# JonathonLuiten/PReMVOS

Measured on AMD Instinct MI355X. Metric: frames/sec (proposal+refine+flow) on 480p DAVIS frames, higher is better.
Workload: dtype f32

## Files before the change

include/premvos_hip.h:

```cpp
#ifndef PREMVOS_HIP_H
#define PREMVOS_HIP_H

#include <stdint.h>

#ifdef __cplusplus
extern "C" {
#endif

#define PREMVOS_OK 0
#define PREMVOS_EINVAL (-1)
#define PREMVOS_ELAUNCH (-2)
#define PREMVOS_EUNSUPPORTED (-3)
#define PREMVOS_ENOSPACE (-4)

#define PREMVOS_ACT_NONE 0
#define PREMVOS_ACT_RELU 1
#define PREMVOS_ACT_LEAKY 2
#define PREMVOS_ACT_SIGMOID 3
#define PREMVOS_ACT_SPLIT8_BF16 0x200

#define PREMVOS_PREC_F32 0
#define PREMVOS_PREC_BF16 1
#define PREMVOS_PREC_BF16X3 3

// ... 37 lines not shown
} premvos_conv_desc;

int premvos_conv2d_f32(const premvos_conv_desc* d, void* stream);
int64_t premvos_conv2d_workspace_bytes(const premvos_conv_desc* d);

int premvos_conv_wino4_slab_f32(const premvos_conv_desc* d, float* vslab, int64_t vslab_bytes, int32_t v_pitch, int32_t v_c0, int32_t t_cn,
                                void* stream);

int premvos_corr_fwd_f32(const float* f1, int32_t f1_ps, const float* f2, int32_t f2_ps, float* out,
                         int32_t out_ps, int32_t n, int32_t h, int32_t w, int32_t c, int32_t md,
                         float slope, int32_t copy_f1, void* stream);

int premvos_corr_nchw_fwd_f32(const float* in1, const float* in2, float* out, int32_t n, int32_t c,
                              int32_t h, int32_t w, int32_t pad_size, int32_t kernel_size,
                              int32_t max_displacement, int32_t stride1, int32_t stride2,
                              int32_t corr_type_multiply, void* stream);

int premvos_warp_fwd_f32(const float* x, int32_t x_ps, const float* flow, int32_t flow_ps, float flow_scale,
                         float* out, int32_t out_ps, int32_t n, int32_t h, int32_t w, int32_t c,
                         void* stream);

int premvos_warp_corr_fwd_f32(const float* f1, int32_t f1_ps, const float* x2, int32_t x2_ps, const float* flow,
                              int32_t flow_ps, float flow_scale, float* out, int32_t out_ps, int32_t n, int32_t h,
                              int32_t w, int32_t c, int32_t md, float slope, int32_t copy_f1, void* stream);

int premvos_nchw_to_nhwc_f32(const float* in, float* out, int32_t out_ps, int32_t n, int32_t c, int32_t h,
                             int32_t w, void* stream);
int premvos_nhwc_to_nchw_f32(const float* in, int32_t in_ps, float* out, int32_t n, int32_t c, int32_t h,
                             int32_t w, void* stream);

int premvos_flow_preprocess_u8(const uint8_t* im1, const uint8_t* im2, int32_t batch, int32_t h, int32_t w,
                               float* out, int32_t h_, int32_t w_, void* stream);
int premvos_flow_postprocess_f32(const float* flow2, int32_t flow_ps, int32_t batch, int32_t h4, int32_t w4,
                                 float* out, int32_t h, int32_t w, int32_t h_, int32_t w_, void* stream);


int premvos_proposal_preprocess_u8(const uint8_t* img_bgr, int32_t batch, int32_t h, int32_t w, float* out,
                                   int32_t nh, int32_t nw, int32_t src_is_rgb, void* stream);

int premvos_maxpool_f32(const float* in, int32_t in_ps, int32_t n, int32_t h, int32_t w, int32_t c, float* out,
                        int32_t out_ps, int32_t ho, int32_t wo, int32_t k, int32_t stride, int32_t pt, int32_t pl,
                        float pad_value, void* stream);

int premvos_rpn_proposals_f32(const float* rpn, int32_t ps, int32_t n, int32_t fh, int32_t fw, int32_t na,
                              int32_t logit_off, int32_t box_off, const float* cell_anchors, float stride,
                              float img_h, float img_w, int32_t pre_nms_topk, int32_t post_nms_topk,
                              float nms_thresh, float min_size, float decode_clip, float* out_boxes,
                              float* out_scores, int32_t* out_idx, int32_t* out_count, void* stream);

int premvos_roi_align_f32(const float* fmap, int32_t fmap_ps, int32_t n_img, int32_t h, int32_t w, int32_t c,
                          const float* rois, const int32_t* count, int32_t rois_per_img, float spatial_scale,
                          int32_t out_size, float* out, int32_t out_ps, void* stream);

int premvos_global_avgpool_f32(const float* in, int32_t in_ps, int32_t n, int32_t hw, int32_t c, float* out,
                               int32_t out_ps, void* stream);

int premvos_frcnn_tail_f32(const float* head, int32_t head_ps, const float* rois, const int32_t* count, int32_t n_img,
                           int32_t rois_per_img, float img_h, float img_w, float score_thresh, float nms_thresh,
                           int32_t max_out, float decode_clip, float rw_x, float rw_y, float rw_w, float rw_h,
                           float* out_boxes, float* out_probs, int32_t* out_idx, int32_t* out_count, void* stream);


int premvos_refine_input_u8(const uint8_t* frame_rgb, int32_t h, int32_t w, const float* boxes_y0x0y1x1,
                            const int32_t* count, int32_t max_boxes, int32_t size, float* out, int32_t* crop_boxes,
                            void* stream);

int premvos_dwconv3x3_f32(const float* in, int32_t in_ps, int32_t n, int32_t h, int32_t w, int32_t c,
                          const float* wgt, const float* bias, int32_t c_pad, float* out, int32_t out_ps, int32_t ho,
                          int32_t wo, int32_t stride, int32_t dilation, int32_t pt, int32_t pl, int32_t pre_relu,
                          int32_t act, void* stream);

#define PREMVOS_DW_TILE 1
#define PREMVOS_DW_ROW 2
#define PREMVOS_DW_PIXEL 3
#define PREMVOS_DW_STORE_F32 0
#define PREMVOS_DW_STORE_S8 1
#define PREMVOS_DW_STORE_S8_PAIRED 2
int premvos_dwconv3x3_variant(int32_t n, int32_t h, int32_t w, int32_t c_pad, int32_t ho, int32_t wo, int32_t stride,
                              int32_t dilation, int32_t pre_relu, int32_t act);

int premvos_conv_bf16x3_s8_f32(const premvos_conv_desc* d, const void* in_s8, const void* wgt_s8, void* out_s8,
                               int32_t out_s8_ps, const void* res_s8, int32_t res_s8_ps, int32_t tile, void* stream);

int premvos_split8_f32(const float* in, int32_t in_ps, void* out_s8, int32_t out_ps, int64_t pixels, int32_t c, void* stream);

int premvos_resize_bilinear_f32(const float* in, int32_t in_ps, int32_t n, int32_t h, int32_t w, int32_t c, float* out,
                                int32_t out_ps, int32_t ho, int32_t wo, int32_t align_corners, void* stream);

int premvos_broadcast_pixel_f32(const float* in, int32_t in_ps, int32_t n, int32_t c, float* out, int32_t out_ps,
                                int32_t h, int32_t w, void* stream);

int64_t premvos_refine_output_workspace_bytes(int32_t max_boxes, int32_t size, int32_t h, int32_t w);
int premvos_refine_output_f32(const float* logits, int32_t logits_ps, int32_t lh, int32_t lw, const int32_t* crop_boxes,
                              const int32_t* count, int32_t max_boxes, int32_t size, int32_t h, int32_t w,
                              uint8_t* mask, float* posterior, float* conf_score, void* workspace, void* stream);

int premvos_mfma_f32_calibrate(int64_t iters, int32_t blocks, float* sink, void* stream);

int premvos_mfma_f32_calibrate_random(int64_t iters, int32_t blocks, float* sink, void* stream);

int premvos_hbm_copy_calibrate(const void* src, void* dst, int64_t n_float4, void* stream);

int premvos_digest_u64(const void* buf, int64_t pixels, int32_t c, int32_t ps, void* out_u64, void* stream);

uint32_t premvos_crc32c_host(const void* data, int64_t n);

// ... 165 lines not shown
```

premvos_amd/_lib.py:

```python
from __future__ import annotations

import ctypes as C
import os

import torch

from . import build as _build

_LIB = None
ABI_VERSION = 21

ACT_NONE, ACT_RELU, ACT_LEAKY, ACT_SIGMOID = 0, 1, 2, 3
MASK_BBOX_SLABS = 16
ACT_SPLIT8_BF16 = 0x200
OUT_NHWC, OUT_PIXSHUF2 = 0, 1
PREC_F32, PREC_BF16, PREC_BF16X3 = 0, 1, 3
PRECISIONS = {"fp32": PREC_F32, "bf16": PREC_BF16, "bf16x3": PREC_BF16X3}


class ConvDesc(C.Structure):
    _fields_ = [
        ("inp", C.c_void_p), ("wgt", C.c_void_p), ("bias", C.c_void_p), ("res", C.c_void_p),
        ("out", C.c_void_p),
        ("n", C.c_int32), ("h", C.c_int32), ("w", C.c_int32), ("cin", C.c_int32),
        ("in_ps", C.c_int32),
        ("ho", C.c_int32), ("wo", C.c_int32), ("cout", C.c_int32),
        ("out_ps", C.c_int32), ("res_ps", C.c_int32),
        ("kh", C.c_int32), ("kw", C.c_int32), ("sh", C.c_int32), ("sw", C.c_int32),
        ("dh", C.c_int32), ("dw", C.c_int32), ("pt", C.c_int32), ("pl", C.c_int32),
        ("cin_pad", C.c_int32), ("k_pad", C.c_int32), ("cout_pad", C.c_int32),
        ("act", C.c_int32), ("slope", C.c_float), ("out_mode", C.c_int32), ("cout_ps", C.c_int32),
        ("tile_hint", C.c_int32), ("split_k", C.c_int32), ("workspace", C.c_void_p), ("workspace_bytes", C.c_int64),
        ("precision", C.c_int32), ("stage_k", C.c_int32), ("wgt_lo", C.c_void_p),
        ("tail_m_tiles", C.c_int32), ("tail_split_k", C.c_int32), ("wgt_wino", C.c_void_p),
        ("wgt_wino4", C.c_void_p),
    ]


_i32, _f32, _vp = C.c_int32, C.c_float, C.c_void_p

SIGNATURES = {
    "premvos_conv2d_f32": [C.POINTER(ConvDesc), _vp],
    "premvos_corr_fwd_f32": [_vp, _i32, _vp, _i32, _vp, _i32, _i32, _i32, _i32, _i32, _i32, _f32, _i32, _vp],
    "premvos_corr_nchw_fwd_f32": [_vp, _vp, _vp, _i32, _i32, _i32, _i32, _i32, _i32, _i32, _i32, _i32, _i32, _vp],
    "premvos_warp_corr_fwd_f32": [_vp, _i32, _vp, _i32, _vp, _i32, _f32, _vp, _i32, _i32, _i32, _i32, _i32, _i32, _f32,
                                  _i32, _vp],
    "premvos_warp_fwd_f32": [_vp, _i32, _vp, _i32, _f32, _vp, _i32, _i32, _i32, _i32, _i32, _vp],
    "premvos_nchw_to_nhwc_f32": [_vp, _vp, _i32, _i32, _i32, _i32, _i32, _vp],
    "premvos_nhwc_to_nchw_f32": [_vp, _i32, _vp, _i32, _i32, _i32, _i32, _vp],
    "premvos_flow_preprocess_u8": [_vp, _vp, _i32, _i32, _i32, _vp, _i32, _i32, _vp],
    "premvos_flow_postprocess_f32": [_vp, _i32, _i32, _i32, _i32, _vp, _i32, _i32, _i32, _i32, _vp],
    "premvos_proposal_preprocess_u8": [_vp, _i32, _i32, _i32, _vp, _i32, _i32, _i32, _vp],
    "premvos_maxpool_f32": [_vp, _i32, _i32, _i32, _i32, _i32, _vp, _i32, _i32, _i32, _i32, _i32, _i32, _i32, _f32, _vp],
    "premvos_rpn_proposals_f32": [_vp, _i32, _i32, _i32, _i32, _i32, _i32, _i32, _vp, _f32, _f32, _f32, _i32, _i32,
                                  _f32, _f32, _f32, _vp, _vp, _vp, _vp, _vp],
    "premvos_roi_align_f32": [_vp, _i32, _i32, _i32, _i32, _i32, _vp, _vp, _i32, _f32, _i32, _vp, _i32, _vp],
    "premvos_global_avgpool_f32": [_vp, _i32, _i32, _i32, _i32, _vp, _i32, _vp],
    "premvos_refine_input_u8": [_vp, _i32, _i32, _vp, _vp, _i32, _i32, _vp, _vp, _vp],
    "premvos_dwconv3x3_f32": [_vp, _i32, _i32, _i32, _i32, _i32, _vp, _vp, _i32, _vp, _i32, _i32, _i32, _i32, _i32,
                              _i32, _i32, _i32, _i32, _vp],
    "premvos_conv_bf16x3_s8_f32": [C.POINTER(ConvDesc), _vp, _vp, _vp, _i32, _vp, _i32, _i32, _vp],
    "premvos_split8_f32": [_vp, _i32, _vp, _i32, C.c_int64, _i32, _vp],
    "premvos_resize_bilinear_f32": [_vp, _i32, _i32, _i32, _i32, _i32, _vp, _i32, _i32, _i32, _i32, _vp],
    "premvos_broadcast_pixel_f32": [_vp, _i32, _i32, _i32, _vp, _i32, _i32, _i32, _vp],
    "premvos_refine_output_f32": [_vp, _i32, _i32, _i32, _vp, _vp, _i32, _i32, _i32, _i32, _vp, _vp, _vp, _vp, _vp],
    "premvos_mfma_f32_calibrate": [C.c_int64, _i32, _vp, _vp],
    "premvos_mfma_f32_calibrate_random": [C.c_int64, _i32, _vp, _vp],
    "premvos_hbm_copy_calibrate": [_vp, _vp, C.c_int64, _vp],
    "premvos_digest_u64": [_vp, C.c_int64, _i32, _i32, _vp, _vp],
    "premvos_conv_wino4_slab_f32": [C.POINTER(ConvDesc), _vp, C.c_int64, _i32, _i32, _i32, _vp],
    "premvos_jpeg_entropy_decode_host": [_vp, C.c_int64, _vp, _vp, C.c_int64],
    "premvos_jpeg_reconstruct_u8": [_vp, _vp, _vp, _vp, _i32, _vp],
    "premvos_overlay_blend_u8": [_vp, _vp, _vp, _i32, _i32, _vp, _vp],
    "premvos_jpeg_forward_u8": [_vp, _vp, _vp, _i32, _i32, _vp, _vp, _i32, _i32, _vp, _vp, C.c_int64, _vp],
    "premvos_jpeg_entropy_encode_host": [_vp, _vp, _vp, C.c_int64, _vp],
    "premvos_reid_input_u8": [_vp, _i32, _i32, _vp, _i32, _i32, _i32, _vp, _vp],
    "premvos_reid_input_frames_u8": [_vp, _i32, _i32, _i32, _vp, _vp, _i32, _i32, _i32, _vp, _vp],
    "premvos_reid_context_boxes_i32": [_vp, _i32, _i32, _i32, _i32, _vp, _vp],
    "premvos_mask_bbox_u8": [_vp, _i32, _i32, _i32, C.c_int64, _i32, _i32, _vp, _vp, _vp, _vp],
    "premvos_scale_shift_relu_f32": [_vp, _i32, C.c_int64, _i32, _vp, _vp, _vp, _i32, _i32, _vp],
    "premvos_mask_warp_u8": [_vp, _i32, _i32, _i32, _vp, _vp, _i32, _vp],
    "premvos_mask_overlap_u8": [_vp, _i32, _vp, _i32, C.c_int64, _vp, _vp, _vp, _vp],
    "premvos_mask_warp_seats_u8": [_vp, _i32, _i32, _i32, _vp, _vp, _i32, _vp, _i32, _vp],
    "premvos_mask_pack_bits_u8": [_vp, C.c_int64, _vp, _vp],
    "premvos_mask_unpack_bits_u8": [_vp, C.c_int64, _vp, _vp],
    "premvos_rle_boundaries_u8": [_vp, _i32, _i32, _i32, _vp, _i32, _vp, _vp, _vp],
    "premvos_rle_boundaries_pooled_u8": [_vp, _i32, _i32, _i32, C.c_int64, _i32, _vp, _i32, _vp, _vp, _vp],
    "premvos_frcnn_tail_f32": [_vp, _i32, _vp, _vp, _i32, _i32, _f32, _f32, _f32, _f32, _i32, _f32, _f32, _f32, _f32,
                               _f32, _vp, _vp, _vp, _vp, _vp],
    "premvos_rle_decode_u8": [_vp, _i32, _vp, _i32, _i32, _i32, _vp, _vp],
    "premvos_track_scores_f64": [_vp, _vp, _vp, _vp, _vp, _vp, _vp, _i32, _i32, _vp, C.c_double, _vp, _vp, _vp, _vp, _vp, _vp],
    "premvos_track_paint_u8": [_vp, _i32, _i32, _i32, _vp, _vp, _vp, _i32, _vp, _vp, _vp, _vp],
    "premvos_track_inputs_f64": [_vp, _vp, _vp, _vp, _i32, _i32, _vp, _vp, _vp],
    "premvos_track_next_f32": [_vp, _vp, _i32, _vp, _vp, _vp],
    "premvos_mask_overlap_seats_u8": [_vp, _i32, C.c_int64, _vp, _i32, _vp, _vp, _vp, _vp],
    "premvos_track_scores_seats_f64": [_vp, _vp, _vp, _vp, _vp, _vp, _vp, _vp, _vp, _i32, _vp, C.c_double, _vp, _vp, _vp, _vp, _vp, _vp],
    "premvos_track_paint_seats_u8": [_vp, _i32, _i32, _i32, _vp, _i32, _vp, _vp, _vp, _vp, _vp, _vp, _i32, _vp, _vp],
    "premvos_track_scores_sets_f64": [_vp, _vp, _vp, _vp, _vp, _vp, _vp, _vp, _vp, _i32, _vp, C.c_double, _vp, _vp, _vp, _vp, _vp, _vp],
    "premvos_track_eval_seats_i64": [_vp, _i32, _i32, _i32, _vp, _i32, _i32, _vp, _vp, C.c_int64, _vp],
    "premvos_mask_label_overlap_u8": [_vp, _i32, _vp, _i32, C.c_int64, _vp, _vp, _vp, _vp],
    "premvos_track_gt_scores_f64": [_vp, _vp, _vp, _i32, _i32, _vp, C.c_double, _vp, _vp, _vp, _vp, _vp, _vp],
    "premvos_track_combine_f64": [_vp, _i32, _i32, _i32, _vp, C.c_int64, _vp, _i32, _vp, _vp, _vp, _vp, _vp, _vp, _vp],
    "premvos_viz_scores_u8": [_vp, _i32, _i32, _vp, _vp, _i32, _vp, _vp, C.c_int64, _vp, _i32, _vp, _vp, C.c_int64, _vp, _vp],
    "premvos_reid_max_distance_f64": [_vp, _i32, _vp, C.c_int64, _vp, _vp, _vp],
    "premvos_davis_counts_u8":[_vp, _vp, _i32, _i32, _i32, _vp, _i32, _i32, _vp, _vp, _vp],
    "premvos_bits_overlap_i32": [_vp, _i32, C.c_int64, C.c_int64, _vp, _vp, _i32, _vp, C.c_int64, _vp, C.c_int64, _vp],
    "premvos_prewarp_reid_f64": [_vp, _vp, _i32, _i32, _vp, _vp, _i32, _vp, _vp, _vp, _vp, _vp],
    "premvos_prewarp_chain_f64": [_vp, C.c_int64, _vp, C.c_int64, _vp, _vp, _vp, _vp, _vp, _vp, _i32, _i32, _vp, _vp, _vp, _vp, _i32, _vp, _vp,
                                  _vp, _vp],
# ... 100 lines not shown
```

premvos_amd/csrc/proposal_ops.hip:

```cpp
#include "common.h"
#include "resize_cv.h"

#pragma clang fp contract(off)

namespace {

__global__ __launch_bounds__(256) void proposal_preprocess_kernel(const uint8_t* __restrict__ img, int batch, int h,
                                                                  int w, float* __restrict__ out, int nh, int nw,
                                                                  int src_is_rgb) {
  const long total = (long)batch * nh * nw;
  const double sx = 1.0 / ((double)nw / (double)w), sy = 1.0 / ((double)nh / (double)h);
  const float mean[3] = {0.406f, 0.456f, 0.485f};
  const float stdv[3] = {0.225f, 0.224f, 0.229f};
  const float inv255 = (float)(1.0 / 255);
  for (long idx = (long)blockIdx.x * 256 + threadIdx.x; idx < total; idx += (long)gridDim.x * 256) {
    const int x = idx % nw, y = (idx / nw) % nh;
    const uint8_t* im = img + (idx / ((long)nw * nh)) * h * w * 3;
    int x0, x1, y0, y1;
    short a0, a1, b0, b1;
    premvos::cv_lin_coef(x, sx, w, &x0, &x1, &a0, &a1);
    premvos::cv_lin_coef(y, sy, h, &y0, &y1, &b0, &b1);
    float px[4];
    for (int ch = 0; ch < 3; ++ch) {
      const int sc = src_is_rgb ? 2 - ch : ch;
// ... 265 lines not shown
    if (rl < count[img]) {
      const float* rb = rois + r * 4;
      const float x0 = rb[0] * scale, y0 = rb[1] * scale, x1 = rb[2] * scale, y1 = rb[3] * scale;
      const float sw = (x1 - x0) / (float)crop, sh = (y1 - y0) / (float)crop;
      const float nx0 = (x0 + sw / 2.f - 0.5f) / (float)(W - 1), ny0 = (y0 + sh / 2.f - 0.5f) / (float)(H - 1);
      const float nw = sw * (float)(crop - 1) / (float)(W - 1), nh = sh * (float)(crop - 1) / (float)(H - 1);
      const float by1 = ny0, bx1 = nx0, by2 = ny0 + nh, bx2 = nx0 + nw;
      const float hs = (by2 - by1) * (float)(H - 1) / (float)(crop - 1);
      const float ws = (bx2 - bx1) * (float)(W - 1) / (float)(crop - 1);
      const float* fb = fm + (long)img * H * W * ps + cg * 4;
      bool oky[2], okx[2];
      int yt[2], yb[2], xl[2], xr[2];
      float yl[2], xlp[2];
#pragma unroll
      for (int j = 0; j < 2; ++j) {
        const float in_y = by1 * (float)(H - 1) + (float)(2 * by_ + j) * hs;
        oky[j] = !(in_y < 0.f || in_y > (float)(H - 1));
        yt[j] = (int)floorf(in_y), yb[j] = (int)ceilf(in_y);
        yl[j] = in_y - floorf(in_y);
        const float in_x = bx1 * (float)(W - 1) + (float)(2 * bx_ + j) * ws;
        okx[j] = !(in_x < 0.f || in_x > (float)(W - 1));
        xl[j] = (int)floorf(in_x), xr[j] = (int)ceilf(in_x);
        xlp[j] = in_x - floorf(in_x);
      }
      float4 tl[2][2], tr[2][2], bl[2][2], br[2][2];
#pragma unroll
      for (int j = 0; j < 2; ++j)
#pragma unroll
        for (int i = 0; i < 2; ++i)
          if (oky[j] && okx[i]) {
            tl[j][i] = *reinterpret_cast<const float4*>(fb + ((long)yt[j] * W + xl[i]) * ps);
            tr[j][i] = *reinterpret_cast<const float4*>(fb + ((long)yt[j] * W + xr[i]) * ps);
            bl[j][i] = *reinterpret_cast<const float4*>(fb + ((long)yb[j] * W + xl[i]) * ps);
            br[j][i] = *reinterpret_cast<const float4*>(fb + ((long)yb[j] * W + xr[i]) * ps);
          }
#pragma unroll
      for (int j = 0; j < 2; ++j)
#pragma unroll
        for (int i = 0; i < 2; ++i)
          if (oky[j] && okx[i]) {
            const float4 a = tl[j][i], b = tr[j][i], c = bl[j][i], d = br[j][i];
            float top, bot;
            top = a.x + (b.x - a.x) * xlp[i]; bot = c.x + (d.x - c.x) * xlp[i]; acc.x += top + (bot - top) * yl[j];
            top = a.y + (b.y - a.y) * xlp[i]; bot = c.y + (d.y - c.y) * xlp[i]; acc.y += top + (bot - top) * yl[j];
            top = a.z + (b.z - a.z) * xlp[i]; bot = c.z + (d.z - c.z) * xlp[i]; acc.z += top + (bot - top) * yl[j];
            top = a.w + (b.w - a.w) * xlp[i]; bot = c.w + (d.w - c.w) * xlp[i]; acc.w += top + (bot - top) * yl[j];
          }
      acc.x *= 0.25f; acc.y *= 0.25f; acc.z *= 0.25f; acc.w *= 0.25f;
    }
    *reinterpret_cast<float4*>(out + ((r * outsz + by_) * outsz + bx_) * out_ps + cg * 4) = acc;
  }
}

__global__ __launch_bounds__(256) void roi_align_row_kernel(const float* __restrict__ fm, int ps, int H, int W, int c4,
                                                            const float* __restrict__ rois, const int* __restrict__ count,
                                                            int rois_per_img, int n_img, float scale, int outsz,
                                                            float* __restrict__ out, int out_ps) {
  const long total = (long)n_img * rois_per_img * outsz * c4;
  const int crop = 2 * outsz;
  for (long idx = (long)blockIdx.x * 256 + threadIdx.x; idx < total; idx += (long)gridDim.x * 256) {
    const int cg = idx % c4;
    long t = idx / c4;
    const int by_ = t % outsz;
    const long r = t / outsz;
    const int img = r / rois_per_img, rl = r % rois_per_img;
    float* orow = out + ((r * outsz + by_) * outsz) * out_ps + cg * 4;
    if (rl >= count[img]) {
      for (int bx_ = 0; bx_ < outsz; ++bx_) *reinterpret_cast<float4*>(orow + (long)bx_ * out_ps) = make_float4(0.f, 0.f, 0.f, 0.f);
      continue;
    }
    const float* rb = rois + r * 4;
    const float x0 = rb[0] * scale, y0 = rb[1] * scale, x1 = rb[2] * scale, y1 = rb[3] * scale;
    const float sw = (x1 - x0) / (float)crop, sh = (y1 - y0) / (float)crop;
    const float nx0 = (x0 + sw / 2.f - 0.5f) / (float)(W - 1), ny0 = (y0 + sh / 2.f - 0.5f) / (float)(H - 1);
    const float nw = sw * (float)(crop - 1) / (float)(W - 1), nh = sh * (float)(crop - 1) / (float)(H - 1);
    const float by1 = ny0, bx1 = nx0, by2 = ny0 + nh, bx2 = nx0 + nw;
    const float hs = (by2 - by1) * (float)(H - 1) / (float)(crop - 1);
    const float ws = (bx2 - bx1) * (float)(W - 1) / (float)(crop - 1);
    const float* fb = fm + (long)img * H * W * ps + cg * 4;
    bool oky[2];
    float yl[2];
    const float* rt[2];
    const float* rbt[2];
#pragma unroll
    for (int j = 0; j < 2; ++j) {
      const float in_y = by1 * (float)(H - 1) + (float)(2 * by_ + j) * hs;
      oky[j] = !(in_y < 0.f || in_y > (float)(H - 1));
      const int yt = oky[j] ? (int)floorf(in_y) : 0, yb = oky[j] ? (int)ceilf(in_y) : 0;
      yl[j] = in_y - floorf(in_y);
      rt[j] = fb + (long)yt * W * ps;
      rbt[j] = fb + (long)yb * W * ps;
    }
    float4 L[2][2], R[2][2];
    int cxl = -2, cxr = -2;
    float4 sv[2][2];
    bool sok[2];
    for (int bx_ = 0; bx_ < outsz; ++bx_) {
#pragma unroll
      for (int i = 0; i < 2; ++i) {
        const int sx = 2 * bx_ + i;
        const float in_x = bx1 * (float)(W - 1) + (float)sx * ws;
        const bool okx = !(in_x < 0.f || in_x > (float)(W - 1));
        sok[i] = okx;
        if (okx) {
          const int xl = (int)floorf(in_x), xr = (int)ceilf(in_x);
          const float xlp = in_x - floorf(in_x);
          if (xl != cxl || xr != cxr) {
            const bool shift = xl == cxr;
#pragma unroll
            for (int j = 0; j < 2; ++j)
              if (oky[j]) {
                if (shift) { L[j][0] = R[j][0]; L[j][1] = R[j][1]; }
                else {
                  L[j][0] = *reinterpret_cast<const float4*>(rt[j] + (long)xl * ps);
                  L[j][1] = *reinterpret_cast<const float4*>(rbt[j] + (long)xl * ps);
                }
                if (xr == xl) { R[j][0] = L[j][0]; R[j][1] = L[j][1]; }
                else {
                  R[j][0] = *reinterpret_cast<const float4*>(rt[j] + (long)xr * ps);
                  R[j][1] = *reinterpret_cast<const float4*>(rbt[j] + (long)xr * ps);
                }
              }
            cxl = xl; cxr = xr;
          }
#pragma unroll
          for (int j = 0; j < 2; ++j)
            if (oky[j]) {
              const float4 a = L[j][0], b = R[j][0], c = L[j][1], d = R[j][1];
              float top, bot;
              top = a.x + (b.x - a.x) * xlp; bot = c.x + (d.x - c.x) * xlp; sv[j][i].x = top + (bot - top) * yl[j];
              top = a.y + (b.y - a.y) * xlp; bot = c.y + (d.y - c.y) * xlp; sv[j][i].y = top + (bot - top) * yl[j];
              top = a.z + (b.z - a.z) * xlp; bot = c.z + (d.z - c.z) * xlp; sv[j][i].z = top + (bot - top) * yl[j];
              top = a.w + (b.w - a.w) * xlp; bot = c.w + (d.w - c.w) * xlp; sv[j][i].w = top + (bot - top) * yl[j];
            }
        }
      }
      float4 acc = make_float4(0.f, 0.f, 0.f, 0.f);
#pragma unroll
      for (int j = 0; j < 2; ++j)
#pragma unroll
        for (int ii = 0; ii < 2; ++ii)
          if (oky[j] && sok[ii]) { acc.x += sv[j][ii].x; acc.y += sv[j][ii].y; acc.z += sv[j][ii].z; acc.w += sv[j][ii].w; }
      acc.x *= 0.25f; acc.y *= 0.25f; acc.z *= 0.25f; acc.w *= 0.25f;
      *reinterpret_cast<float4*>(orow + (long)bx_ * out_ps) = acc;
    }
  }
}

__global__ __launch_bounds__(256) void gap_kernel(const float* __restrict__ in, int in_ps, int n, int hw, int c4,
                                                  float* __restrict__ out, int out_ps) {
  const long total = (long)n * c4;
  for (long idx = (long)blockIdx.x * 256 + threadIdx.x; idx < total; idx += (long)gridDim.x * 256) {
    const int cg = idx % c4;
    const long b = idx / c4;
    float4 s = make_float4(0.f, 0.f, 0.f, 0.f);
    for (int i = 0; i < hw; ++i) {
      const float4 v = *reinterpret_cast<const float4*>(in + (b * hw + i) * in_ps + cg * 4);
      s.x += v.x; s.y += v.y; s.z += v.z; s.w += v.w;
    }
    const float inv = (float)hw;
    *reinterpret_cast<float4*>(out + b * out_ps + cg * 4) = make_float4(s.x / inv, s.y / inv, s.z / inv, s.w / inv);
  }
}

__global__ __launch_bounds__(256) void gap_sliced_kernel(const float* __restrict__ in, int in_ps, int hw, int c4,
                                                         float* __restrict__ out, int out_ps) {
  __shared__ float4 part[8][32];
  const int lane = threadIdx.x & 31, slice = threadIdx.x >> 5;
  const int cg = blockIdx.x * 32 + lane;
  const long b = blockIdx.y;
  float4 s = make_float4(0.f, 0.f, 0.f, 0.f);
  if (cg < c4) {
    const float* base = in + b * hw * (long)in_ps + cg * 4;
    for (int i = slice; i < hw; i += 8) {
      const float4 v = *reinterpret_cast<const float4*>(base + (long)i * in_ps);
      s.x += v.x; s.y += v.y; s.z += v.z; s.w += v.w;
    }
  }
  part[slice][lane] = s;
  __syncthreads();
  if (slice == 0 && cg < c4) {
#pragma unroll
    for (int k = 1; k < 8; ++k) {
      const float4 v = part[k][lane];
      s.x += v.x; s.y += v.y; s.z += v.z; s.w += v.w;
    }
    const float inv = (float)hw;
    *reinterpret_cast<float4*>(out + b * out_ps + cg * 4) = make_float4(s.x / inv, s.y / inv, s.z / inv, s.w / inv);
  }
}

constexpr int TAIL_NT = 128;

struct TailArgs {
  const float* head;
  int ps, rois_per_img;
  const float* rois;
// ... 85 lines not shown
}

extern "C" int premvos_maxpool_f32(const float* in, int32_t in_ps, int32_t n, int32_t h, int32_t w, int32_t c,
                                   float* out, int32_t out_ps, int32_t ho, int32_t wo, int32_t k, int32_t stride,
                                   int32_t pt, int32_t pl, float pad_value, void* stream) {
  PV_REQUIRE(in && out, "maxpool: null pointer");
  PV_REQUIRE(n > 0 && h > 0 && w > 0 && c > 0 && ho > 0 && wo > 0 && k > 0 && stride > 0, "maxpool: bad dims");
  PV_REQUIRE(c % 4 == 0 && in_ps % 4 == 0 && out_ps % 4 == 0 && in_ps >= c && out_ps >= c,
             "maxpool: C and pixel strides must be multiples of 4");
  PV_REQUIRE(premvos::aligned16(in) && premvos::aligned16(out), "maxpool: in/out must be 16-byte aligned");
  hipLaunchKernelGGL(maxpool_kernel, dim3(grid_for((long)n * ho * wo * (c / 4))), dim3(256), 0,
                     static_cast<hipStream_t>(stream), in, in_ps, n, h, w, c / 4, out, out_ps, ho, wo, k, stride, pt,
                     pl, pad_value);
  return premvos::check_launch("maxpool");
}

extern "C" int premvos_rpn_proposals_f32(const float* rpn, int32_t ps, int32_t n, int32_t fh, int32_t fw, int32_t na,
                                         int32_t logit_off, int32_t box_off, const float* cell_anchors, float stride,
                                         float img_h, float img_w, int32_t pre_nms_topk, int32_t post_nms_topk,
                                         float nms_thresh, float min_size, float decode_clip, float* out_boxes,
                                         float* out_scores, int32_t* out_idx, int32_t* out_count, void* stream) {
  PV_REQUIRE(rpn && cell_anchors && out_boxes && out_scores && out_idx && out_count, "rpn_proposals: null pointer");
  PV_REQUIRE(n > 0 && fh > 0 && fw > 0 && na > 0, "rpn_proposals: bad dims");
  PV_REQUIRE(ps >= logit_off + na && ps >= box_off + 4 * na && logit_off >= 0 && box_off >= 0,
             "rpn_proposals: channel window exceeds pixel stride");
  PV_REQUIRE(pre_nms_topk > 0 && pre_nms_topk <= RPN_NT, "rpn_proposals: pre_nms_topk must be in [1,%d]", RPN_NT);
  PV_REQUIRE(post_nms_topk > 0 && post_nms_topk <= 128, "rpn_proposals: post_nms_topk must be in [1,128]");
  PV_REQUIRE((long)fh * fw * na < (1L << 31), "rpn_proposals: too many anchors");
  RpnArgs a;
  a.rpn = rpn; a.ps = ps; a.fh = fh; a.fw = fw; a.na = na; a.logit_off = logit_off; a.box_off = box_off;
  a.cell_anchors = cell_anchors; a.stride = stride; a.img_h = img_h; a.img_w = img_w; a.nms_thresh = nms_thresh;
  a.min_size = min_size; a.decode_clip = decode_clip; a.pre_k = pre_nms_topk; a.post_k = post_nms_topk;
  a.out_boxes = out_boxes; a.out_scores = out_scores; a.out_idx = out_idx; a.out_count = out_count;
  hipLaunchKernelGGL(rpn_proposals_kernel, dim3(n), dim3(RPN_NT), 0, static_cast<hipStream_t>(stream), a);
  return premvos::check_launch("rpn_proposals");
}

extern "C" int premvos_roi_align_f32(const float* fmap, int32_t fmap_ps, int32_t n_img, int32_t h, int32_t w,
                                     int32_t c, const float* rois, const int32_t* count, int32_t rois_per_img,
                                     float spatial_scale, int32_t out_size, float* out, int32_t out_ps, void* stream) {
  PV_REQUIRE(fmap && rois && count && out, "roi_align: null pointer");
  PV_REQUIRE(n_img > 0 && h > 1 && w > 1 && c > 0 && rois_per_img > 0 && out_size > 0, "roi_align: bad dims");
  PV_REQUIRE(c % 4 == 0 && fmap_ps % 4 == 0 && out_ps % 4 == 0 && fmap_ps >= c && out_ps >= c,
             "roi_align: C and pixel strides must be multiples of 4");
  PV_REQUIRE(premvos::aligned16(fmap) && premvos::aligned16(out), "roi_align: fmap/out must be 16-byte aligned");
  static const bool per_bin = [] { const char* e = getenv("PREMVOS_ROI_ALIGN"); return e != nullptr && e[0] == 'b'; }();
  if (per_bin) {
    const long total = (long)n_img * rois_per_img * out_size * out_size * (c / 4);
    hipLaunchKernelGGL(roi_align_kernel, dim3(grid_for(total)), dim3(256), 0,
                       static_cast<hipStream_t>(stream), fmap, fmap_ps, h, w, c / 4, rois, count, rois_per_img, n_img,
                       spatial_scale, out_size, out, out_ps);
  } else {
    const long total = (long)n_img * rois_per_img * out_size * (c / 4);
    hipLaunchKernelGGL(roi_align_row_kernel, dim3(grid_for(total)), dim3(256), 0,
                       static_cast<hipStream_t>(stream), fmap, fmap_ps, h, w, c / 4, rois, count, rois_per_img, n_img,
                       spatial_scale, out_size, out, out_ps);
  }
  return premvos::check_launch("roi_align");
}

extern "C" int premvos_global_avgpool_f32(const float* in, int32_t in_ps, int32_t n, int32_t hw, int32_t c, float* out,
                                          int32_t out_ps, void* stream) {
  PV_REQUIRE(in && out, "global_avgpool: null pointer");
  PV_REQUIRE(n > 0 && hw > 0 && c > 0, "global_avgpool: bad dims");
  PV_REQUIRE(c % 4 == 0 && in_ps % 4 == 0 && out_ps % 4 == 0 && in_ps >= c && out_ps >= c,
             "global_avgpool: C and strides must be multiples of 4");
  PV_REQUIRE(premvos::aligned16(in) && premvos::aligned16(out), "global_avgpool: in/out must be 16-byte aligned");
  if (hw >= 128) {
    hipLaunchKernelGGL(gap_sliced_kernel, dim3((c / 4 + 31) / 32, n), dim3(256), 0, static_cast<hipStream_t>(stream), in,
                       in_ps, hw, c / 4, out, out_ps);
  } else {
    hipLaunchKernelGGL(gap_kernel, dim3(grid_for((long)n * (c / 4))), dim3(256), 0, static_cast<hipStream_t>(stream),
                       in, in_ps, n, hw, c / 4, out, out_ps);
  }
  return premvos::check_launch("global_avgpool");
}

extern "C" int premvos_frcnn_tail_f32(const float* head, int32_t head_ps, const float* rois, const int32_t* count,
                                      int32_t n_img, int32_t rois_per_img, float img_h, float img_w,
                                      float score_thresh, float nms_thresh, int32_t max_out, float decode_clip,
                                      float rw_x, float rw_y, float rw_w, float rw_h, float* out_boxes,
                                      float* out_probs, int32_t* out_idx, int32_t* out_count, void* stream) {
  PV_REQUIRE(head && rois && count && out_boxes && out_probs && out_idx && out_count, "frcnn_tail: null pointer");
  PV_REQUIRE(rw_x > 0.f && rw_y > 0.f && rw_w > 0.f && rw_h > 0.f, "frcnn_tail: bad regression weights");
  PV_REQUIRE(n_img > 0 && rois_per_img > 0 && rois_per_img <= TAIL_NT, "frcnn_tail: rois_per_img must be in [1,%d]",
             TAIL_NT);
  PV_REQUIRE(head_ps >= 6 && max_out > 0 && max_out <= 64, "frcnn_tail: bad head_ps/max_out");
  TailArgs a;
  a.head = head; a.ps = head_ps; a.rois_per_img = rois_per_img; a.rois = rois; a.count = count;
  a.img_h = img_h; a.img_w = img_w; a.score_thresh = score_thresh; a.nms_thresh = nms_thresh;
  a.decode_clip = decode_clip;
  a.rw0 = rw_x; a.rw1 = rw_y; a.rw2 = rw_w; a.rw3 = rw_h;
  a.max_out = max_out; a.out_boxes = out_boxes; a.out_probs = out_probs; a.out_idx = out_idx; a.out_count = out_count;
  hipLaunchKernelGGL(frcnn_tail_kernel, dim3(n_img), dim3(TAIL_NT), 0, static_cast<hipStream_t>(stream), a);
  return premvos::check_launch("frcnn_tail");
}
```

premvos_amd/proposal/model.py:

```python
from __future__ import annotations

import math
from typing import Dict, Optional, Sequence, Tuple

import numpy as np
import torch

from .. import _lib, arena, ops
from ..ops import ACT_NONE, ACT_RELU, ACT_SIGMOID, NHWC
from ..plan import LaunchPlan

RESNET_NUM_BLOCK = (3, 4, 23, 3)
ANCHOR_STRIDE = 16
ANCHOR_SIZES = (32, 64, 128, 256, 512)
ANCHOR_RATIOS = (0.5, 1.0, 2.0)
NUM_ANCHOR = 15
MAX_SIZE = 1333
BBOX_DECODE_CLIP = float(np.float32(np.log(MAX_SIZE / 16.0)))
TEST_PRE_NMS_TOPK, TEST_POST_NMS_TOPK = 1000, 100
RPN_PROPOSAL_NMS_THRESH, RPN_MIN_SIZE = 0.7, 0.0
FASTRCNN_BBOX_REG_WEIGHTS = (10.0, 10.0, 5.0, 5.0)
FASTRCNN_NMS_THRESH, RESULT_SCORE_THRESH, RESULTS_PER_IM = 0.5, 0.5, 20
NUM_CLASS, SECOND_NUM_CLASS = 2, 81
BN_EPS = 1e-5


def cell_anchors() -> np.ndarray:
    base = ANCHOR_STRIDE
    scales = np.array(ANCHOR_SIZES, np.float64) / base
    out = []
    w = h = float(base)
    xc = yc = 0.5 * (base - 1)
    for r in ANCHOR_RATIOS:
        ws = np.round(np.sqrt(w * h / r))
        hs = np.round(ws * r)
        for s in scales:
            sw, sh = ws * s, hs * s
            out.append([xc - 0.5 * (sw - 1), yc - 0.5 * (sh - 1), xc + 0.5 * (sw - 1), yc + 0.5 * (sh - 1)])
    a = np.array(out, np.float32)
    a[:, 2:] += 1
    return a


def _fold_bn(bn: Dict[str, torch.Tensor]) -> Tuple[torch.Tensor, torch.Tensor]:
    scale = bn["gamma"].double() / torch.sqrt(bn["var"].double() + BN_EPS)
    bias = bn["beta"].double() - bn["mean"].double() * scale
    return scale.float(), bias.float()


class _Plan(LaunchPlan):
    def __init__(self, net: "ProposalNet", b: int, h: int, w: int):
        dev = net.device
        self.b, self.h, self.w = b, h, w
        self.arena = arena.two_pass(dev, lambda A: self._build(net, b, h, w, A))
        self.tune(dev)

    def _build(self, net: "ProposalNet", b: int, h: int, w: int, A: "arena.Arena"):
        self.reset()
        P, lib = net.packed, _lib.load()

        def alloc(n, hh, ww, c):
            ps = (c + 3) // 4 * 4
            return NHWC(A.alloc(n, hh, ww, ps, "f32", pooled=ps == c), c=c)

        S8 = net.packed_s8

        def alloc_s8(n, hh, ww, c):
            assert c % 8 == 0
            return NHWC(A.alloc(n, hh, ww, c, "s8"), c=c, layout="s8")

        def release(*vs):
            for v in vs:
                if v is not None:
                    A.release(v)

        def conv(x, name, out, uid=None, **kw):
            self.conv(uid or name, x, (S8 if x.layout == "s8" else P)[name], out, **kw)

        self.img = alloc(b, h, w, 3)
        h0, w0 = ops.out_size(h, 7, 2, 2, 3), ops.out_size(w, 7, 2, 2, 3)
        c0 = alloc(b, h0, w0, 64)
        conv(self.img, "conv0", c0, stride=(2, 2), pad=(2, 2), act=ACT_RELU)
        hp, wp = ops.out_size(h0, 3, 2, 0, 1), ops.out_size(w0, 3, 2, 0, 1)
        x = alloc(b, hp, wp, 64)

        def pool(i=c0, o=x):
            _lib.check(lib.premvos_maxpool_f32(i.ptr, i.ps, i.n, i.h, i.w, i.c, o.ptr, o.ps, o.h, o.w, 3, 2, 0, 0,
                                               0.0, _lib.current_stream()), "maxpool")
        self.add("maxpool", pool)
        release(c0)

        def group(x: Optional[NHWC], g: int, feat: int, count: int, stride: int, tag: str = "", x8: Optional[NHWC] = None,
                  last_s8: bool = False, last_f32: bool = True):
            s8 = net.s8 and g >= net.s8_from
            shape = (x if x is not None else x8)
            n_, h_, w_, c_ = shape.n, shape.h, shape.w, shape.c
            own_x = own_x8 = False
            for i in range(count):
                p = f"group{g}/block{i}"
                s = stride if i == 0 else 1
                last = i + 1 == count
                if s8 and x8 is None:
                    x8 = alloc_s8(n_, h_, w_, c_)
                    own_x8 = True
                    self.add(f"split8:{tag}{p}", lambda i_=x, o_=x8: ops.split8(i_, o_))
                xin = x8 if s8 else x
                mk = alloc_s8 if s8 else alloc
                t1 = mk(n_, h_, w_, feat)
                o1 = dict(out=None, out_s8=t1) if s8 else dict(out=t1)
                conv(xin, p + "/conv1", uid=tag + p + "/conv1", act=ACT_RELU, **o1)
                if s == 2:
                    ho, wo = ops.out_size(h_, 3, 2, 0, 1), ops.out_size(w_, 3, 2, 0, 1)
                    t2 = mk(n_, ho, wo, feat)
                    o2 = dict(out=None, out_s8=t2) if s8 else dict(out=t2)
                    conv(t1, p + "/conv2", uid=tag + p + "/conv2", stride=(2, 2), pad=(0, 0), act=ACT_RELU, **o2)
                else:
                    ho, wo = h_, w_
                    t2 = mk(n_, h_, w_, feat)
                    o2 = dict(out=None, out_s8=t2) if s8 else dict(out=t2)
                    conv(t1, p + "/conv2", uid=tag + p + "/conv2", pad=(1, 1), act=ACT_RELU, **o2)
                res, res8 = x, None
                if p + "/convshortcut" in P or p + "/convshortcut" in S8:
                    res = alloc(n_, ho, wo, feat * 4)
                    conv(xin, p + "/convshortcut", res, uid=tag + p + "/convshortcut", stride=(s, s))
                elif s8:
                    res, res8 = None, x8
                want_f32 = not s8 or (last and last_f32)
                y = alloc(n_, ho, wo, feat * 4) if want_f32 else None
                y8 = alloc_s8(n_, ho, wo, feat * 4) if s8 and (not last or last_s8) else None
                conv(t2, p + "/conv3", y, uid=tag + p + "/conv3", out_s8=y8, res=res, res_s8=res8, act=ACT_RELU)
                release(t1, t2, res if res is not x else None, x if own_x else None, x8 if own_x8 else None)
                x, x8, h_, w_, c_, own_x, own_x8 = y, y8, ho, wo, feat * 4, True, True
            return x, x8

        nb = net.num_blocks
        s8g = [net.s8 and g >= net.s8_from for g in range(4)]
        x1, x18 = group(x, 0, 64, nb[0], 1, last_s8=s8g[1], last_f32=not s8g[1])
        release(x)
        x2, x28 = group(x1, 1, 128, nb[1], 2, x8=x18, last_s8=s8g[2], last_f32=not s8g[2])
        release(x1, x18)
        fm, fm8 = group(x2, 2, 256, nb[2], 2, x8=x28, last_s8=net.s8 and net.s8_rpn)
        release(x2, x28)
        self.featuremap = fm
        fh, fw = fm.h, fm.w
        hid = alloc(b, fh, fw, 1024)
        conv(fm8 if fm8 is not None else fm, "rpn/conv0", hid, pad=(1, 1), act=ACT_RELU)
        release(fm8)
        self.rpn_out = alloc(b, fh, fw, 5 * NUM_ANCHOR)
        conv(hid, "rpn/heads", self.rpn_out)
        release(hid)
        R = TEST_POST_NMS_TOPK
        self.rois = A.side((b, R, 4), torch.float32)
        self.roi_scores = A.side((b, R), torch.float32)
        self.roi_idx = A.side((b, R), torch.int32)
        self.roi_count = A.side((b,), torch.int32)
        ca = net.cell_anchors_dev

        def rpn(o=self.rpn_out):
            _lib.check(lib.premvos_rpn_proposals_f32(
                o.ptr, o.ps, b, fh, fw, NUM_ANCHOR, 0, NUM_ANCHOR, ca.data_ptr(), float(ANCHOR_STRIDE), float(h),
                float(w), TEST_PRE_NMS_TOPK, R, RPN_PROPOSAL_NMS_THRESH, RPN_MIN_SIZE, BBOX_DECODE_CLIP,
                self.rois.data_ptr(), self.roi_scores.data_ptr(), self.roi_idx.data_ptr(), self.roi_count.data_ptr(),
                _lib.current_stream()), "rpn_proposals")
        self.add("rpn_proposals", rpn)
        roi = alloc(b * R, 14, 14, 1024)

        def ralign(o=roi):
            _lib.check(lib.premvos_roi_align_f32(fm.ptr, fm.ps, b, fh, fw, 1024, self.rois.data_ptr(),
                                                 self.roi_count.data_ptr(), R, 1.0 / ANCHOR_STRIDE, 14, o.ptr, o.ps,
                                                 _lib.current_stream()), "roi_align")
        self.add("roi_align", ralign)
        f5, _ = group(roi, 3, 512, nb[3], 2)
        release(roi)
        self.feat5 = f5
        gp = alloc(b * R, 1, 1, 2048)

        def gap(i=f5, o=gp):
            _lib.check(lib.premvos_global_avgpool_f32(i.ptr, i.ps, i.n, i.h * i.w, i.c, o.ptr, o.ps,
                                                      _lib.current_stream()), "gap")
        self.add("global_avgpool", gap)
        nh = NUM_CLASS + 4 * (NUM_CLASS - 1) + SECOND_NUM_CLASS
        self.head = alloc(b * R, 1, 1, nh)
        conv(gp, "heads", self.head)
        M = RESULTS_PER_IM
        self.final_boxes = A.side((b, M, 4), torch.float32)
        self.final_probs = A.side((b, M), torch.float32)
        self.final_idx = A.side((b, M), torch.int32)
        self.final_count = A.side((b,), torch.int32)

        def tail(hd=self.head):
            _lib.check(lib.premvos_frcnn_tail_f32(
                hd.ptr, hd.ps, self.rois.data_ptr(), self.roi_count.data_ptr(), b, R, float(h), float(w),
                RESULT_SCORE_THRESH, FASTRCNN_NMS_THRESH, M, BBOX_DECODE_CLIP, *FASTRCNN_BBOX_REG_WEIGHTS,
                self.final_boxes.data_ptr(), self.final_probs.data_ptr(), self.final_idx.data_ptr(),
                self.final_count.data_ptr(), _lib.current_stream()), "frcnn_tail")
        self.add("frcnn_tail", tail)

        self.final_masks: Optional[NHWC] = None
        if net.mode_mask:
            mroi = alloc(b * M, 14, 14, 1024)

            def malign(o=mroi):
                _lib.check(lib.premvos_roi_align_f32(fm.ptr, fm.ps, b, fh, fw, 1024, self.final_boxes.data_ptr(),
                                                     self.final_count.data_ptr(), M, 1.0 / ANCHOR_STRIDE, 14, o.ptr,
                                                     o.ps, _lib.current_stream()), "roi_align(mask)")
            self.add("roi_align_mask", malign)
            mf5, _ = group(mroi, 3, 512, nb[3], 2, tag="mask:")
            release(mroi)
            up = alloc(b * M, 14, 14, 256)
            conv(mf5, "maskrcnn/deconv", up, act=ACT_RELU)
            release(mf5)
            self.final_masks = alloc(b * M, 14, 14, NUM_CLASS - 1)
            conv(up, "maskrcnn/conv", self.final_masks, act=ACT_SIGMOID)
            release(up)


class ProposalNet:

    def __init__(self, weights: Dict[str, object], num_blocks: Sequence[int] = RESNET_NUM_BLOCK,
                 device=None, use_graph: bool = True, precision: Optional[str] = None,
                 mode_mask: bool = False):
        _lib.require_gpu()
        self.mode_mask = mode_mask
        self.precision = prec = precision or ops.default_precision()
        self.device, self.use_graph, self.num_blocks = _lib.resolve_device(device), use_graph, tuple(num_blocks)
        device = self.device
        self.packed: Dict[str, ops.PackedConv] = {}
        self._plans: Dict[tuple, _Plan] = {}
        self.cell_anchors_dev = torch.from_numpy(cell_anchors()).to(device)
        w = weights
        import os
        self.s8 = prec == "bf16x3" and os.environ.get("PREMVOS_BF16X3_SPLIT", "1") != "0"
        self.s8_from = int(os.environ.get("PREMVOS_BF16X3_S8_FROM", "1"))
        self.packed_s8: Dict[str, ops.PackedConvS8] = {}
        for name in [k[:-2] for k in w if k.endswith("/W") and (k[:-2] + "/bn") in w]:
            scale, bias = _fold_bn(w[name + "/bn"])
            if self.s8 and name.startswith("group") and int(name[5]) >= self.s8_from:
                self.packed_s8[name] = ops.pack_conv_s8(w[name + "/W"], bias, device, scale=scale)
            else:
                self.packed[name] = ops.pack_conv(w[name + "/W"], bias, device, scale=scale, precision="fp32" if self.s8 else prec)
        self.s8_rpn = os.environ.get("PREMVOS_S8_RPN", "0") == "1"
        if self.s8 and self.s8_rpn:
            self.packed_s8["rpn/conv0"] = ops.pack_conv_s8(w["rpn/conv0/W"], w["rpn/conv0/b"], device)
        else:
            self.packed["rpn/conv0"] = ops.pack_conv(w["rpn/conv0/W"], w["rpn/conv0/b"], device, precision="fp32" if self.s8 else prec)
        self.packed["rpn/heads"] = ops.pack_conv(torch.cat([w["rpn/class/W"], w["rpn/box/W"]], 0),
                                                 torch.cat([w["rpn/class/b"], w["rpn/box/b"]], 0), device, precision=prec)
        hw = torch.cat([w["fastrcnn/class/W"], w["fastrcnn/box/W"], w["secondclassification/class/W"]], 0)
        hb = torch.cat([w["fastrcnn/class/b"], w["fastrcnn/box/b"], w["secondclassification/class/b"]], 0)
        self.packed["heads"] = ops.pack_conv(hw.view(hw.shape[0], hw.shape[1], 1, 1), hb, device, precision=prec)
        if mode_mask:
            self.packed["maskrcnn/deconv"] = ops.pack_deconv2x2s2(w["maskrcnn/deconv/W"], w["maskrcnn/deconv/b"], device,
                                                                  precision=prec)
            self.packed["maskrcnn/conv"] = ops.pack_conv(w["maskrcnn/conv/W"], w["maskrcnn/conv/b"], device, precision=prec)

    def plan(self, b: int, h: int, w: int) -> _Plan:
        key = (b, h, w)
        if key not in self._plans:
            if h // ANCHOR_STRIDE < 2 or w // ANCHOR_STRIDE < 2:
                raise ValueError("image too small for the stride-16 feature map")
            p = _Plan(self, b, h, w)
            if self.use_graph:
                p.capture()
            self._plans[key] = p
        return self._plans[key]

    def run_resized(self, img_bgr: torch.Tensor) -> _Plan:
        b, h, w, _ = img_bgr.shape
        p = self.plan(b, h, w)
        _lib.check(_lib.load().premvos_proposal_preprocess_u8(img_bgr.contiguous().data_ptr(), b, h, w, p.img.ptr, h,
                                                              w, 0, _lib.current_stream()), "proposal_preprocess")
        p.launch()
        return p

    def outputs(self, p: _Plan, i: int = 0):
        n = int(p.final_count[i].item())
        boxes = p.final_boxes[i, :n].cpu().numpy()
        probs = p.final_probs[i, :n].cpu().numpy()
        idx = p.final_idx[i, :n].cpu().numpy().astype(np.int64)
        labels = np.ones((n,), np.int64)
        head = p.head.buf.view(p.b, TEST_POST_NMS_TOPK, -1)[i].cpu().numpy()
        cls = head[:, :2]
        e = np.exp(cls - cls.max(1, keepdims=True))
        label_probs = e / e.sum(1, keepdims=True)
        final_posterior = label_probs[np.zeros((n,), np.int64)] if n else np.zeros((0, 2), np.float32)
        sec = head[:, 6:6 + SECOND_NUM_CLASS]
        es = np.exp(sec - sec.max(1, keepdims=True))
        sec_probs = es / es.sum(1, keepdims=True)
        second_final_posterior = sec_probs[np.zeros((n,), np.int64)] if n else np.zeros((0, SECOND_NUM_CLASS), np.float32)
        second_final_labels = (final_posterior.argmax(-1) + 1) if n else np.zeros((0,), np.int64)
        return boxes, probs, labels, final_posterior, second_final_labels, second_final_posterior, idx

    def masks(self, p: _Plan, i: int = 0) -> np.ndarray:
# ... 4 lines not shown
```

Measured before the change: 54.26.

## Commute group3 block0 1x1 conv and shortcut sampling ahead of ROI align

```diff
diff --git a/include/premvos_hip.h b/include/premvos_hip.h
--- a/include/premvos_hip.h
+++ b/include/premvos_hip.h
@@ -113,6 +113,11 @@
                           const float* rois, const int32_t* count, int32_t rois_per_img, float spatial_scale,
                           int32_t out_size, float* out, int32_t out_ps, void* stream);
 
+int premvos_roi_align_epi_f32(const float* fmap, int32_t fmap_ps, int32_t n_img, int32_t h, int32_t w, int32_t c,
+                              const float* rois, const int32_t* count, int32_t rois_per_img, float spatial_scale,
+                              int32_t out_size, int32_t bin_step, const float* bias, int32_t act, float* out,
+                              int32_t out_ps, void* stream);
+
 int premvos_global_avgpool_f32(const float* in, int32_t in_ps, int32_t n, int32_t hw, int32_t c, float* out,
                                int32_t out_ps, void* stream);
 
diff --git a/premvos_amd/_lib.py b/premvos_amd/_lib.py
--- a/premvos_amd/_lib.py
+++ b/premvos_amd/_lib.py
@@ -55,6 +55,8 @@
     "premvos_rpn_proposals_f32": [_vp, _i32, _i32, _i32, _i32, _i32, _i32, _i32, _vp, _f32, _f32, _f32, _i32, _i32,
                                   _f32, _f32, _f32, _vp, _vp, _vp, _vp, _vp],
     "premvos_roi_align_f32": [_vp, _i32, _i32, _i32, _i32, _i32, _vp, _vp, _i32, _f32, _i32, _vp, _i32, _vp],
+    "premvos_roi_align_epi_f32": [_vp, _i32, _i32, _i32, _i32, _i32, _vp, _vp, _i32, _f32, _i32, _i32, _vp, _i32, _vp, _i32,
+                                  _vp],
     "premvos_global_avgpool_f32": [_vp, _i32, _i32, _i32, _i32, _vp, _i32, _vp],
     "premvos_refine_input_u8": [_vp, _i32, _i32, _vp, _vp, _i32, _i32, _vp, _vp, _vp],
     "premvos_dwconv3x3_f32": [_vp, _i32, _i32, _i32, _i32, _i32, _vp, _vp, _i32, _vp, _i32, _i32, _i32, _i32, _i32,
diff --git a/premvos_amd/csrc/proposal_ops.hip b/premvos_amd/csrc/proposal_ops.hip
--- a/premvos_amd/csrc/proposal_ops.hip
+++ b/premvos_amd/csrc/proposal_ops.hip
@@ -341,21 +341,34 @@
   }
 }
 
+template <bool EPI, int STEP>
 __global__ __launch_bounds__(256) void roi_align_row_kernel(const float* __restrict__ fm, int ps, int H, int W, int c4,
                                                             const float* __restrict__ rois, const int* __restrict__ count,
                                                             int rois_per_img, int n_img, float scale, int outsz,
+                                                            const float* __restrict__ bias, int act,
                                                             float* __restrict__ out, int out_ps) {
-  const long total = (long)n_img * rois_per_img * outsz * c4;
+  const int on = (outsz + STEP - 1) / STEP;
+  const long total = (long)n_img * rois_per_img * on * c4;
   const int crop = 2 * outsz;
   for (long idx = (long)blockIdx.x * 256 + threadIdx.x; idx < total; idx += (long)gridDim.x * 256) {
     const int cg = idx % c4;
     long t = idx / c4;
-    const int by_ = t % outsz;
-    const long r = t / outsz;
+    const int oy = t % on, by_ = oy * STEP;
+    const long r = t / on;
     const int img = r / rois_per_img, rl = r % rois_per_img;
-    float* orow = out + ((r * outsz + by_) * outsz) * out_ps + cg * 4;
+    float* orow = out + ((r * on + oy) * on) * out_ps + cg * 4;
+    float4 bv = make_float4(0.f, 0.f, 0.f, 0.f);
+    if (EPI && bias != nullptr) bv = *reinterpret_cast<const float4*>(bias + cg * 4);
+    auto epilogue = [&](float4 v) {
+      if (EPI) {
+        v.x = __fadd_rn(v.x, bv.x); v.y = __fadd_rn(v.y, bv.y); v.z = __fadd_rn(v.z, bv.z); v.w = __fadd_rn(v.w, bv.w);
+        if (act == PREMVOS_ACT_RELU) { v.x = fmaxf(v.x, 0.f); v.y = fmaxf(v.y, 0.f); v.z = fmaxf(v.z, 0.f); v.w = fmaxf(v.w, 0.f); }
+      }
+      return v;
+    };
     if (rl >= count[img]) {
-      for (int bx_ = 0; bx_ < outsz; ++bx_) *reinterpret_cast<float4*>(orow + (long)bx_ * out_ps) = make_float4(0.f, 0.f, 0.f, 0.f);
+      const float4 z = epilogue(make_float4(0.f, 0.f, 0.f, 0.f));
+      for (int ox = 0; ox < on; ++ox) *reinterpret_cast<float4*>(orow + (long)ox * out_ps) = z;
       continue;
     }
     const float* rb = rois + r * 4;
@@ -384,7 +397,7 @@
     int cxl = -2, cxr = -2;
     float4 sv[2][2];
     bool sok[2];
-    for (int bx_ = 0; bx_ < outsz; ++bx_) {
+    for (int bx_ = 0; bx_ < outsz; bx_ += STEP) {
 #pragma unroll
       for (int i = 0; i < 2; ++i) {
         const int sx = 2 * bx_ + i;
@@ -431,7 +444,7 @@
         for (int ii = 0; ii < 2; ++ii)
           if (oky[j] && sok[ii]) { acc.x += sv[j][ii].x; acc.y += sv[j][ii].y; acc.z += sv[j][ii].z; acc.w += sv[j][ii].w; }
       acc.x *= 0.25f; acc.y *= 0.25f; acc.z *= 0.25f; acc.w *= 0.25f;
-      *reinterpret_cast<float4*>(orow + (long)bx_ * out_ps) = acc;
+      *reinterpret_cast<float4*>(orow + (long)(bx_ / STEP) * out_ps) = epilogue(acc);
     }
   }
 }
@@ -623,11 +636,35 @@
                        spatial_scale, out_size, out, out_ps);
   } else {
     const long total = (long)n_img * rois_per_img * out_size * (c / 4);
-    hipLaunchKernelGGL(roi_align_row_kernel, dim3(grid_for(total)), dim3(256), 0,
+    hipLaunchKernelGGL((roi_align_row_kernel<false, 1>), dim3(grid_for(total)), dim3(256), 0,
                        static_cast<hipStream_t>(stream), fmap, fmap_ps, h, w, c / 4, rois, count, rois_per_img, n_img,
-                       spatial_scale, out_size, out, out_ps);
+                       spatial_scale, out_size, static_cast<const float*>(nullptr), PREMVOS_ACT_NONE, out, out_ps);
   }
   return premvos::check_launch("roi_align");
+}
+
+extern "C" int premvos_roi_align_epi_f32(const float* fmap, int32_t fmap_ps, int32_t n_img, int32_t h, int32_t w,
+                                         int32_t c, const float* rois, const int32_t* count, int32_t rois_per_img,
+                                         float spatial_scale, int32_t out_size, int32_t bin_step, const float* bias,
+                                         int32_t act, float* out, int32_t out_ps, void* stream) {
+  PV_REQUIRE(fmap && rois && count && out, "roi_align_epi: null pointer");
+  PV_REQUIRE(n_img > 0 && h > 1 && w > 1 && c > 0 && rois_per_img > 0 && out_size > 0, "roi_align_epi: bad dims");
+  PV_REQUIRE(c % 4 == 0 && fmap_ps % 4 == 0 && out_ps % 4 == 0 && fmap_ps >= c && out_ps >= c,
+             "roi_align_epi: C and pixel strides must be multiples of 4");
+  PV_REQUIRE(premvos::aligned16(fmap) && premvos::aligned16(out) && premvos::aligned16(bias),
+             "roi_align_epi: fmap/out/bias must be 16-byte aligned");
+  PV_REQUIRE(bin_step == 1 || bin_step == 2, "roi_align_epi: bin_step must be 1 or 2");
+  PV_REQUIRE(act == PREMVOS_ACT_NONE || act == PREMVOS_ACT_RELU, "roi_align_epi: act must be none or ReLU");
+  const int on = (out_size + bin_step - 1) / bin_step;
+  const long total = (long)n_img * rois_per_img * on * (c / 4);
+  const bool epi = bias != nullptr || act != PREMVOS_ACT_NONE;
+#define PV_ROI_EPI(E, S)                                                                                                \
+  hipLaunchKernelGGL((roi_align_row_kernel<E, S>), dim3(grid_for(total)), dim3(256), 0, static_cast<hipStream_t>(stream), \
+                     fmap, fmap_ps, h, w, c / 4, rois, count, rois_per_img, n_img, spatial_scale, out_size, bias, act, out, out_ps)
+  if (bin_step == 1) { if (epi) PV_ROI_EPI(true, 1); else PV_ROI_EPI(false, 1); }
+  else { if (epi) PV_ROI_EPI(true, 2); else PV_ROI_EPI(false, 2); }
+#undef PV_ROI_EPI
+  return premvos::check_launch("roi_align_epi");
 }
 
 extern "C" int premvos_global_avgpool_f32(const float* in, int32_t in_ps, int32_t n, int32_t hw, int32_t c, float* out,
diff --git a/premvos_amd/proposal/model.py b/premvos_amd/proposal/model.py
--- a/premvos_amd/proposal/model.py
+++ b/premvos_amd/proposal/model.py
@@ -1,5 +1,6 @@
 from __future__ import annotations
 
+import dataclasses
 import math
 from typing import Dict, Optional, Sequence, Tuple
 
@@ -91,9 +92,10 @@
         release(c0)
 
         def group(x: Optional[NHWC], g: int, feat: int, count: int, stride: int, tag: str = "", x8: Optional[NHWC] = None,
-                  last_s8: bool = False, last_f32: bool = True):
+                  last_s8: bool = False, last_f32: bool = True, pre: Optional[Tuple[NHWC, NHWC]] = None):
             s8 = net.s8 and g >= net.s8_from
-            shape = (x if x is not None else x8)
+            assert pre is None or (not s8 and x is None and x8 is None)
+            shape = pre[0] if pre is not None else (x if x is not None else x8)
             n_, h_, w_, c_ = shape.n, shape.h, shape.w, shape.c
             own_x = own_x8 = False
             for i in range(count):
@@ -106,9 +108,13 @@
                     self.add(f"split8:{tag}{p}", lambda i_=x, o_=x8: ops.split8(i_, o_))
                 xin = x8 if s8 else x
                 mk = alloc_s8 if s8 else alloc
-                t1 = mk(n_, h_, w_, feat)
-                o1 = dict(out=None, out_s8=t1) if s8 else dict(out=t1)
-                conv(xin, p + "/conv1", uid=tag + p + "/conv1", act=ACT_RELU, **o1)
+                xs = None
+                if pre is not None and i == 0:
+                    t1, xs = pre
+                else:
+                    t1 = mk(n_, h_, w_, feat)
+                    o1 = dict(out=None, out_s8=t1) if s8 else dict(out=t1)
+                    conv(xin, p + "/conv1", uid=tag + p + "/conv1", act=ACT_RELU, **o1)
                 if s == 2:
                     ho, wo = ops.out_size(h_, 3, 2, 0, 1), ops.out_size(w_, 3, 2, 0, 1)
                     t2 = mk(n_, ho, wo, feat)
@@ -122,14 +128,17 @@
                 res, res8 = x, None
                 if p + "/convshortcut" in P or p + "/convshortcut" in S8:
                     res = alloc(n_, ho, wo, feat * 4)
-                    conv(xin, p + "/convshortcut", res, uid=tag + p + "/convshortcut", stride=(s, s))
+                    if xs is not None:
+                        conv(xs, p + "/convshortcut", res, uid=tag + p + "/convshortcut")
+                    else:
+                        conv(xin, p + "/convshortcut", res, uid=tag + p + "/convshortcut", stride=(s, s))
                 elif s8:
                     res, res8 = None, x8
                 want_f32 = not s8 or (last and last_f32)
                 y = alloc(n_, ho, wo, feat * 4) if want_f32 else None
                 y8 = alloc_s8(n_, ho, wo, feat * 4) if s8 and (not last or last_s8) else None
                 conv(t2, p + "/conv3", y, uid=tag + p + "/conv3", out_s8=y8, res=res, res_s8=res8, act=ACT_RELU)
-                release(t1, t2, res if res is not x else None, x if own_x else None, x8 if own_x8 else None)
+                release(t1, t2, xs, res if res is not x else None, x if own_x else None, x8 if own_x8 else None)
                 x, x8, h_, w_, c_, own_x, own_x8 = y, y8, ho, wo, feat * 4, True, True
             return x, x8
 
@@ -149,6 +158,11 @@
         self.rpn_out = alloc(b, fh, fw, 5 * NUM_ANCHOR)
         conv(hid, "rpn/heads", self.rpn_out)
         release(hid)
+        PROJ = "group3/block0/conv1/proj"
+        gproj = None
+        if PROJ in P:
+            gproj = alloc(b, fh, fw, 512)
+            conv(fm, PROJ, gproj)
         R = TEST_POST_NMS_TOPK
         self.rois = A.side((b, R, 4), torch.float32)
         self.roi_scores = A.side((b, R), torch.float32)
@@ -163,15 +177,30 @@
                 self.rois.data_ptr(), self.roi_scores.data_ptr(), self.roi_idx.data_ptr(), self.roi_count.data_ptr(),
                 _lib.current_stream()), "rpn_proposals")
         self.add("rpn_proposals", rpn)
-        roi = alloc(b * R, 14, 14, 1024)
-
-        def ralign(o=roi):
-            _lib.check(lib.premvos_roi_align_f32(fm.ptr, fm.ps, b, fh, fw, 1024, self.rois.data_ptr(),
-                                                 self.roi_count.data_ptr(), R, 1.0 / ANCHOR_STRIDE, 14, o.ptr, o.ps,
-                                                 _lib.current_stream()), "roi_align")
-        self.add("roi_align", ralign)
-        f5, _ = group(roi, 3, 512, nb[3], 2)
-        release(roi)
+
+        def ralign_epi(name, i, o, step, bias, act):
+            bp = bias.data_ptr() if bias is not None else None
+            self.add("roi_align_epi:" + name, lambda: _lib.check(lib.premvos_roi_align_epi_f32(
+                i.ptr, i.ps, b, fh, fw, i.c, self.rois.data_ptr(), self.roi_count.data_ptr(), R, 1.0 / ANCHOR_STRIDE, 14, step, bp,
+                act, o.ptr, o.ps, _lib.current_stream()), "roi_align_epi:" + name))
+
+        if gproj is not None:
+            t1 = alloc(b * R, 14, 14, 512)
+            ralign_epi("group3/block0/conv1", gproj, t1, 1, P["group3/block0/conv1"].bias, ACT_RELU)
+            release(gproj)
+            roi_s = alloc(b * R, 7, 7, 1024)
+            ralign_epi("group3/block0/convshortcut", fm, roi_s, 2, None, ACT_NONE)
+            f5, _ = group(None, 3, 512, nb[3], 2, pre=(t1, roi_s))
+        else:
+            roi = alloc(b * R, 14, 14, 1024)
+
+            def ralign(o=roi):
+                _lib.check(lib.premvos_roi_align_f32(fm.ptr, fm.ps, b, fh, fw, 1024, self.rois.data_ptr(),
+                                                     self.roi_count.data_ptr(), R, 1.0 / ANCHOR_STRIDE, 14, o.ptr, o.ps,
+                                                     _lib.current_stream()), "roi_align")
+            self.add("roi_align", ralign)
+            f5, _ = group(roi, 3, 512, nb[3], 2)
+            release(roi)
         self.feat5 = f5
         gp = alloc(b * R, 1, 1, 2048)
 
@@ -239,6 +268,9 @@
                 self.packed_s8[name] = ops.pack_conv_s8(w[name + "/W"], bias, device, scale=scale)
             else:
                 self.packed[name] = ops.pack_conv(w[name + "/W"], bias, device, scale=scale, precision="fp32" if self.s8 else prec)
+        c1 = self.packed.get("group3/block0/conv1")
+        if c1 is not None and c1.precision == _lib.PREC_F32:
+            self.packed["group3/block0/conv1/proj"] = dataclasses.replace(c1, bias=None)
         self.s8_rpn = os.environ.get("PREMVOS_S8_RPN", "0") == "1"
         if self.s8 and self.s8_rpn:
             self.packed_s8["rpn/conv0"] = ops.pack_conv_s8(w["rpn/conv0/W"], w["rpn/conv0/b"], device)
```

New measurement: 55.04 (median of 6 runs). 1.01x the previous value.
